# claymore666/openhush

Measured on AMD Instinct MI355X. Metric: audio-sec/sec (xRT) large-v3 greedy, 30s chunks, 1/2/4/8 MI355X, higher is better.
Workload: dtype bf16; 1 GPU; large-v3 dims, steps of batch=32 x 30 s windows per GPU, greedy, 100 tokens/window (EOT suppressed), procedural weights seed 1234, every window a distinct synthetic recording, PCM resident in HBM; schedule LANES 4x3: 12 steps (384 windows) in flight per GPU - per lane ONE front-end pass and ONE decode batch of 96 rows, 4 decodes side by side on 64 CUs each; concurrent_sub_batches=1

## Files before the change

### include/ohw.h

```cpp
#ifndef OHW_H
#define OHW_H

#include <stddef.h>
#include <stdint.h>

#ifdef __cplusplus
extern "C" {
#endif

#define OHW_ABI_VERSION 2

enum {
  OHW_OK = 0,
  OHW_E_MODEL_NOT_FOUND = -3001,
  OHW_E_LOAD_FAILED = -3002,
  OHW_E_TRANSCRIBE = -3003,
  OHW_E_NO_GPU = -3004,
  OHW_E_OOM = -3005,
  OHW_E_INVALID_ARG = -3006,
  OHW_E_VALIDATION = -3007
};

enum { OHW_DTYPE_AUTO = -1, OHW_DTYPE_BF16 = 0, OHW_DTYPE_F16 = 1 };

// ... 512 lines not shown
  void* x16_out;
  float* stat_out;
  void* k_cache;
  void* v_cache;
  const int32_t* n_past;
  int32_t d_model, n_head, n_ctx;
  int32_t* shape_out;
} ohw_dbg_dec_gemm_io;
int ohw_dbg_dec_gemm(const ohw_dbg_dec_gemm_io* io, void* stream);
int ohw_dbg_embed(int dtype, const float* emb, int n_vocab, const float* pos, int n_pos, const int32_t* tok_host,
                  const int32_t* n_past_host, float* x, void* x16, float* stat, int M, int n_new, int d, void* stream);
int ohw_dbg_layernorm(int dtype, const float* x, const float* gamma, const float* beta, void* y, int64_t rows, int d, int tiled,
                      void* stream);

enum { OHW_EG_KERNEL_AUTO = 0, OHW_EG_KERNEL_K128, OHW_EG_KERNEL_SMALL, OHW_EG_KERNEL_K256 };
typedef struct {
  int32_t dtype, epilogue, kernel;
  int32_t conv_cin;
  int64_t M, N, K;
  int64_t lda, a_batch_stride, rows_per_batch;
  int64_t ldc, c_batch_stride;
  int32_t d_model, n_head, t_len, batch, batch_offset;
  const int32_t* c_row_map;
  const void* a;
  int64_t a_elems;
  const float* w;
  const float* bias;
  const float* pos;
  void* out;
  int64_t out_elems;
} ohw_dbg_enc_gemm_io;
int ohw_dbg_enc_gemm(const ohw_dbg_enc_gemm_io* io, void* stream);

#ifdef __cplusplus
}
#endif
#endif
```

### openhush_amd/csrc/engine.hip

```cpp
#include <execinfo.h>
#include <signal.h>
#include <unistd.h>

#include <cstring>
#include <memory>
#include <mutex>
#include <shared_mutex>
#include <type_traits>
#include <vector>
#include <algorithm>

#include "attention.hpp"
#include "dequant.hpp"
#include "gemm.hpp"
#include "kernels.hpp"
#include "model.hpp"

namespace ohw {
ohw_ctx* ctx_from_file(const char* path, int device, int dtype);
ohw_ctx* ctx_synthetic(const ohw_hparams* hp, uint32_t seed, int device, int dtype);
ohw_ctx* ctx_shell(const ohw_hparams* hp, int device, int dtype);
void select_device(int device);

thread_local std::string g_last_error;
// ... 3180 lines not shown
      const int64_t need = (nb - 1) * a.c_batch_stride + (rows - 1) * a.ldc + a.N;
      if (need > a.out_elems) bad("the output rows end at element " + str(need) + ", past out_elems = " + str(a.out_elems));
      if (a.epilogue == EPI_GELU_POS_F32 && (!a.pos || !aligned16(a.pos))) bad("GELU_POS_F32 needs pos, 16-byte aligned");
    }

    hipStream_t s = (hipStream_t)stream;
    DevBuf wt, map;
    wt.alloc((size_t)a.N * a.K * 2);
    if (a.c_row_map) dbg_upload(map, a.c_row_map, (size_t)a.M);
    Dispatch::run(a.dtype, [&](auto* tag) {
      using TT = std::remove_pointer_t<decltype(tag)>;
      if (a.conv_cin > 0) launch_repack_conv<TT>(a.w, wt.p, a.N, a.conv_cin, a.K / 3, s);
      else launch_convert_rows<TT>(a.w, wt.p, a.N, a.K, a.K, s);
      GemmParams g{};
      g.A = a.a; g.W = wt.p; g.bias = a.bias; g.out = a.out; g.pos = a.epilogue == EPI_GELU_POS_F32 ? a.pos : nullptr;
      g.M = a.M; g.N = a.N; g.K = a.K;
      g.lda = a.lda; g.a_batch_stride = a.a_batch_stride; g.rows_per_batch = a.rows_per_batch;
      g.ldc = a.ldc; g.c_batch_stride = a.c_batch_stride;
      if (a.epilogue == EPI_CROSSKV_T) {
        g.d_model = a.d_model; g.n_head = a.n_head; g.t_len = a.t_len; g.batch = a.batch; g.batch_offset = a.batch_offset;
        g.c_row_map = a.c_row_map ? map.as<int32_t>() : nullptr;
      }
      switch (a.kernel) {
        case OHW_EG_KERNEL_K128: launch_gemm128<TT>(g, a.epilogue, s); break;
        case OHW_EG_KERNEL_SMALL: launch_gemm_small<TT>(g, a.epilogue, s); break;
        case OHW_EG_KERNEL_K256: launch_gemm256<TT>(g, a.epilogue, s); break;
        default: launch_gemm<TT>(g, a.epilogue, s); break;
      }
    });
    HIP_CHECK(hipStreamSynchronize(s));
  });
}

}
```

### openhush_amd/csrc/gemm.hpp

```cpp
#pragma once
#include "common.hpp"

namespace ohw {

enum GemmEpilogue {
  EPI_BIAS_T = 0,
  EPI_BIAS_GELU_T = 1,
  EPI_BIAS_RESID_F32 = 2,
  EPI_GELU_POS_F32 = 3,
  EPI_F32 = 4,
  EPI_CROSSKV_T = 5
};

struct GemmParams {
  const void* A;
  const void* W;
  const float* bias;
  void* out;
  const float* pos;
  int64_t M, N, K;
  int64_t lda, a_batch_stride, rows_per_batch;
  int64_t ldc, c_batch_stride;
  int32_t d_model, n_head, t_len, batch;
  int32_t batch_offset;
  int32_t group_m;
  int32_t small_m;
  const int32_t* c_row_map;
};

template <typename T> void launch_gemm(const GemmParams& p, int epilogue, hipStream_t stream);
template <typename T> void launch_gemm128(const GemmParams& p, int epilogue, hipStream_t stream);
template <typename T> void launch_gemm_small(const GemmParams& p, int epilogue, hipStream_t stream);
template <typename T> void launch_gemm256(const GemmParams& p, int epilogue, hipStream_t stream);

}
```

### openhush_amd/csrc/gemm256.hip

```cpp
#include <algorithm>
#include <cstdlib>

#include "gemm.hpp"
#include "gemm_epilogue.hpp"

namespace ohw {

constexpr int G2_BM = 256, G2_BN = 256, G2_BK = 64;
constexpr int G2_THREADS = 512;
constexpr int G2_OPSTAGE = 32768;
constexpr int G2_NA = 3;
constexpr int G2_WBASE = G2_NA * G2_OPSTAGE;
constexpr int G2_LDS = G2_WBASE + 2 * G2_OPSTAGE;

__device__ __forceinline__ int g2_key(int row) { return (row >> 1) & 7; }

#ifdef OHW_TRACE
constexpr unsigned G2_TRACE_CAP = 1u << 16;
__device__ unsigned long long g2_trace_buf[G2_TRACE_CAP * 12];
__device__ unsigned g2_trace_n;
#define G2T(k) do { if (tid == 0 && g2_slot < G2_TRACE_CAP) g2_trace_buf[g2_slot * 12 + (k)] = wall_clock64(); } while (0)
#else
#define G2T(k) do { } while (0)
#endif

template <typename T, int EPI>
__global__ __launch_bounds__(G2_THREADS, 2) void gemm256_kernel(GemmParams p) {
  using Ops = TypeOps<T>;
  using vec8 = typename Ops::vec8;
  extern __shared__ __attribute__((aligned(16))) unsigned char smem[];
  const int tid = threadIdx.x;
  const int lane = tid & 63;
  const int wave = __builtin_amdgcn_readfirstlane(tid >> 6);
  const int wm = wave >> 2, wn = wave & 3;
#ifdef OHW_TRACE
  unsigned g2_slot = G2_TRACE_CAP;
  if (tid == 0) {
    g2_slot = atomicAdd(&g2_trace_n, 1u);
    if (g2_slot < G2_TRACE_CAP) {
      unsigned hw, xcc;
      asm volatile("s_getreg_b32 %0, hwreg(HW_REG_HW_ID)" : "=s"(hw));
      asm volatile("s_getreg_b32 %0, hwreg(HW_REG_XCC_ID)" : "=s"(xcc));
      g2_trace_buf[g2_slot * 12 + 0] = blockIdx.x;
      g2_trace_buf[g2_slot * 12 + 1] = ((unsigned long long)(xcc & 0xf) << 32) | hw;
    }
  }
  G2T(2);
#endif

  const unsigned n_tiles_n = (unsigned)(p.N / G2_BN);
  const unsigned n_tiles_m = (unsigned)((p.M + G2_BM - 1) / G2_BM);
  const unsigned nwg = n_tiles_n * n_tiles_m;
  const T* __restrict__ A = (const T*)p.A;
  const T* __restrict__ W = (const T*)p.W;

  const int sr = lane >> 3, sc = lane & 7;
  unsigned a_off[4], w_off[4];
  int64_t m0 = 0, n0 = 0;
  auto tile_setup = [&](unsigned d) {
    const unsigned lid = xcd_remap(d, nwg);
    const unsigned GM = (unsigned)p.group_m;
    const unsigned per_group = GM * n_tiles_n;
    const unsigned grp_id = lid / per_group, in_grp = lid % per_group;
    const unsigned g_first = grp_id * GM;
    const unsigned g_size = n_tiles_m - g_first < GM ? n_tiles_m - g_first : GM;
    m0 = (int64_t)(g_first + in_grp % g_size) * G2_BM;
    n0 = (int64_t)(in_grp / g_size) * G2_BN;
#pragma unroll
    for (int j = 0; j < 4; ++j) {
      const int R = (wave * 4 + j) * 8 + sr;
      const int dchunk = sc ^ g2_key(R);
      int64_t m = m0 + R;
      if (m > p.M - 1) m = p.M - 1;
      int64_t b = 0, rr = m;
      if (p.rows_per_batch < p.M) { const unsigned bb = (unsigned)m / (unsigned)p.rows_per_batch; b = bb; rr = m - (int64_t)bb * p.rows_per_batch; }
      a_off[j] = (unsigned)((b * p.a_batch_stride + rr * p.lda + dchunk * 8) * 2);
      const int rl = R & 63;
      const int nl = (((rl >> 2) & 3) << 4) + ((rl >> 4) << 2) + (rl & 3);
      w_off[j] = (unsigned)(((n0 + (R & ~63) + nl) * p.K + dchunk * 8) * 2);
    }
  };
  const int KT = (int)(p.K / G2_BK);

  auto issue_A = [&](int kt) {
    const unsigned koff = (unsigned)(kt * G2_BK * 2);
    const int buf = (kt % G2_NA) * G2_OPSTAGE;
#pragma unroll
    for (int j = 0; j < 4; ++j)
      __builtin_amdgcn_global_load_lds((const __attribute__((address_space(1))) void*)((const char*)A + (size_t)(a_off[j] + koff)),
                                       (__attribute__((address_space(3))) void*)(smem + buf + (wave * 4 + j) * 1024), 16, 0, 0);
  };
  auto issue_W = [&](int kt) {
    const unsigned koff = (unsigned)(kt * G2_BK * 2);
// ... 23 lines not shown
#pragma unroll
    for (int ni = 0; ni < 4; ++ni) fw[ni] = *(const vec8*)(smem + wcur + w_row + ch + ni * 2048);
#pragma unroll
    for (int mi = 0; mi < 8; ++mi) fa[mi] = *(const vec8*)(smem + acur + a_row + ch + mi * 2048);
  };
  auto compute = [&]() {
    __builtin_amdgcn_s_setprio(1);
#pragma unroll
    for (int mi = 0; mi < 8; ++mi)
#pragma unroll
      for (int ni = 0; ni < 4; ++ni) acc[mi][ni] = Ops::mfma16(fw[ni], fa[mi], acc[mi][ni]);
    __builtin_amdgcn_s_setprio(0);
  };
  auto open_even = [&](int Pn) {
    if (Pn < NP && (Pn & 1) == 0) {
      if ((Pn >> 1) + 1 < KT) asm volatile("s_waitcnt vmcnt(4)" ::: "memory");
      else asm volatile("s_waitcnt vmcnt(0)" ::: "memory");
    }
    asm volatile("s_waitcnt lgkmcnt(0)" ::: "memory");
    __builtin_amdgcn_s_barrier();
    __builtin_amdgcn_sched_barrier(0);
  };
  auto open_odd = [&]() {
    asm volatile("s_waitcnt lgkmcnt(0)" ::: "memory");
    __builtin_amdgcn_s_barrier();
    __builtin_amdgcn_sched_barrier(0);
  };
  auto raw_barrier = [&]() {
    asm volatile("s_waitcnt lgkmcnt(0)" ::: "memory");
    __builtin_amdgcn_s_barrier();
    __builtin_amdgcn_sched_barrier(0);
  };

  const unsigned d = blockIdx.x;
  tile_setup(d);
  issue_A(0); issue_W(0);
  if (KT > 1) issue_A(1);
  {
    const int64_t m0c = m0, n0c = n0;
    const int64_t nb = n0c + wn * 64 + fq * 16;
    f32x4 bias4[4] = {{0.f, 0.f, 0.f, 0.f}, {0.f, 0.f, 0.f, 0.f}, {0.f, 0.f, 0.f, 0.f}, {0.f, 0.f, 0.f, 0.f}};
    if (p.bias) {
#pragma unroll
      for (int j = 0; j < 4; ++j) bias4[j] = *(const f32x4*)(p.bias + nb + 4 * j);
    }
#pragma unroll
    for (int i = 0; i < 8; ++i)
#pragma unroll
      for (int j = 0; j < 4; ++j) acc[i][j] = (f32x4){0.f, 0.f, 0.f, 0.f};

    if (wm == 0) {
      for (int P = 0; P < NP; ++P) {
        open_even(P);
#ifdef OHW_TRACE
        if (P == 0) G2T(3);
#endif
        read_frags(P);
        if ((P & 1) == 0) issue_ahead(P >> 1);
        __builtin_amdgcn_sched_barrier(0);
        open_odd();
        compute();
        __builtin_amdgcn_sched_barrier(0);
      }
      open_even(NP);
    } else {
      open_even(0);
      for (int P = 0; P < NP; ++P) {
        open_odd();
        read_frags(P);
        if ((P & 1) == 0) issue_ahead(P >> 1);
        __builtin_amdgcn_sched_barrier(0);
        open_even(P + 1);
        compute();
        __builtin_amdgcn_sched_barrier(0);
      }
    }
    G2T(4);

    int lane_e = lane;
    asm volatile("" : "+v"(lane_e));
    const int fr_e = lane_e & 15, fq_e = lane_e >> 4;
    float bias[16];
#pragma unroll
    for (int j = 0; j < 16; ++j) bias[j] = bias4[j >> 2][j & 3];
    bool stored = false;
    if constexpr (EPI == EPI_BIAS_RESID_F32) {
      float* outf = (float*)p.out;
      auto row_ptr = [&](int r, int i) -> float* {
        int64_t m = m0c + (wave >> 2) * 128 + r * 64 + (wave & 3) * 16 + i;
        if (m > p.M - 1) m = p.M - 1;
        int64_t bb = 0, rr = m;
        if (p.rows_per_batch < p.M) { const unsigned q = (unsigned)m / (unsigned)p.rows_per_batch; bb = q; rr = m - (int64_t)q * p.rows_per_batch; }
        return outf + bb * p.c_batch_stride + rr * p.ldc + n0c + lane_e * 4;
      };
      auto to_lds = [&](int r) {
#pragma unroll
        for (int q = 0; q < 4; ++q) {
          const int row = wm * 64 + q * 16 + fr_e;
#pragma unroll
          for (int ni = 0; ni < 4; ++ni) {
            const int chunk = (wn * 16 + fq_e * 4 + ni) ^ (row & 15);
            f32x4 v4 = acc[4 * r + q][ni];
            v4.x += bias[4 * ni]; v4.y += bias[4 * ni + 1]; v4.z += bias[4 * ni + 2]; v4.w += bias[4 * ni + 3];
            *(f32x4*)(smem + row * 1024 + chunk * 16) = v4;
          }
        }
      };
      f32x4 old0[16], old1[16];
#pragma unroll
      for (int i = 0; i < 16; ++i) old0[i] = *(const f32x4*)row_ptr(0, i);
      G2T(6);
      to_lds(0);
      raw_barrier();
      G2T(7);
#pragma unroll
      for (int i = 0; i < 16; ++i) old1[i] = *(const f32x4*)row_ptr(1, i);
#pragma unroll
      for (int i = 0; i < 16; ++i) {
        const int lr = wave * 16 + i;
        if (m0c + (wave >> 2) * 128 + (wave & 3) * 16 + i >= p.M) continue;
        const f32x4 v4 = *(const f32x4*)(smem + lr * 1024 + ((lane_e ^ (lr & 15)) << 4));
        f32x4 o4 = old0[i];
        o4.x += v4.x; o4.y += v4.y; o4.z += v4.z; o4.w += v4.w;
        *(f32x4*)row_ptr(0, i) = o4;
      }
      G2T(8);
      raw_barrier();
      to_lds(1);
      raw_barrier();
      G2T(9);
      f32x4 v1[16];
#pragma unroll
      for (int i = 0; i < 16; ++i) {
        const int lr = wave * 16 + i;
        v1[i] = *(const f32x4*)(smem + lr * 1024 + ((lane_e ^ (lr & 15)) << 4));
      }
#pragma unroll
      for (int i = 0; i < 16; ++i) {
        if (m0c + (wave >> 2) * 128 + 64 + (wave & 3) * 16 + i >= p.M) continue;
        f32x4 o4 = old1[i];
        o4.x += v1[i].x; o4.y += v1[i].y; o4.z += v1[i].z; o4.w += v1[i].w;
        *(f32x4*)row_ptr(1, i) = o4;
      }
      G2T(10);
      G2T(11);
      stored = true;
    }
    if constexpr (EPI == EPI_BIAS_T || EPI == EPI_BIAS_GELU_T) {
      {
        G2T(9);
#pragma unroll
        for (int mi = 0; mi < 8; ++mi) {
          const int row = wm * 128 + mi * 16 + fr_e;
          float v[16];
#pragma unroll
          for (int ni = 0; ni < 4; ++ni)
#pragma unroll
            for (int j = 0; j < 4; ++j) v[ni * 4 + j] = acc[mi][ni][j] + bias[ni * 4 + j];
          if constexpr (EPI == EPI_BIAS_GELU_T) {
#pragma unroll
            for (int j = 0; j < 16; ++j) v[j] = gelu_erf(v[j]);
          }
          u32x4 lo, hi;
          lo.x = pack2<T>(v[0], v[1]); lo.y = pack2<T>(v[2], v[3]); lo.z = pack2<T>(v[4], v[5]); lo.w = pack2<T>(v[6], v[7]);
          hi.x = pack2<T>(v[8], v[9]); hi.y = pack2<T>(v[10], v[11]); hi.z = pack2<T>(v[12], v[13]); hi.w = pack2<T>(v[14], v[15]);
          const int c0 = wn * 8 + fq_e * 2;
          *(u32x4*)(smem + row * 512 + ((c0 ^ fr_e) << 4)) = lo;
          *(u32x4*)(smem + row * 512 + (((c0 + 1) ^ fr_e) << 4)) = hi;
        }
        G2T(7);
        raw_barrier();
        G2T(8);
        T* outp = (T*)p.out;
#pragma unroll
        for (int half = 0; half < 2; ++half) {
#pragma unroll
          for (int i = 0; i < 8; ++i) {
            const int r = half * 128 + wave * 16 + 2 * i + (lane_e >> 5);
            const int64_t m = m0c + r;
            if (m >= p.M) continue;
            int64_t bb = 0, rr = m;
            if (p.rows_per_batch < p.M) { const unsigned q = (unsigned)m / (unsigned)p.rows_per_batch; bb = q; rr = m - (int64_t)q * p.rows_per_batch; }
            const u32x4 d4 = *(const u32x4*)(smem + r * 512 + (((lane_e & 31) ^ (r & 15)) << 4));
            *(u32x4*)(outp + bb * p.c_batch_stride + rr * p.ldc + n0c + (lane_e & 31) * 8) = d4;
          }
        }
        stored = true;
      }
    }
    if (!stored) {
#pragma unroll
      for (int mi = 0; mi < 8; ++mi) {
        const int64_t m = m0c + wm * 128 + mi * 16 + fr_e;
        if (m >= p.M) continue;
        float v[16];
#pragma unroll
        for (int ni = 0; ni < 4; ++ni)
#pragma unroll
          for (int j = 0; j < 4; ++j) v[ni * 4 + j] = acc[mi][ni][j] + bias[ni * 4 + j];
        gemm_store_row<T, EPI>(p, m, n0c + wn * 64 + fq_e * 16, v);
      }
    }
#ifdef OHW_TRACE
    G2T(6 + (EPI == EPI_BIAS_RESID_F32 ? 5 : 0));
    asm volatile("s_waitcnt vmcnt(0)" ::: "memory");
    G2T(5);
#endif
  }
}

template <typename T, int EPI>
static void launch256_one(const GemmParams& p, hipStream_t stream) {
  const unsigned nwg = (unsigned)((p.N / G2_BN) * ((p.M + G2_BM - 1) / G2_BM));
  ensure_dynamic_lds((const void*)gemm256_kernel<T, EPI>, G2_LDS);
  GemmParams q = p;
  static const int gm_env = [] { const char* e = getenv("OHW_GEMM_GM"); return e ? atoi(e) : 0; }();
  q.group_m = gm_env > 0 ? gm_env : 6;
  hipLaunchKernelGGL((gemm256_kernel<T, EPI>), dim3(nwg), dim3(G2_THREADS), G2_LDS, stream, q);
  HIP_CHECK(hipGetLastError());
}

template <typename T>
void launch_gemm256(const GemmParams& p, int epilogue, hipStream_t stream) {
  if (p.M <= 0) return;
  if (p.N % G2_BN != 0 || p.K % G2_BK != 0 || p.lda % 8 != 0 || p.a_batch_stride % 8 != 0 || p.rows_per_batch <= 0 || p.M >= ((int64_t)1 << 31) || p.N >= ((int64_t)1 << 31))
    throw Error(OHW_E_INVALID_ARG, "gemm256: N must be a multiple of 256, K of 64, row strides of 8 elements");
  {
    const int64_t nb_ = (p.M + p.rows_per_batch - 1) / p.rows_per_batch;
    const int64_t a_bytes = ((nb_ - 1) * p.a_batch_stride + (std::min(p.M, p.rows_per_batch) + 2) * p.lda + p.K) * 2, w_bytes = p.N * p.K * 2;
    if (a_bytes >= ((int64_t)1 << 32) || w_bytes >= ((int64_t)1 << 32)) throw Error(OHW_E_INVALID_ARG, "gemm256: an operand spans 4 GiB or more");
  }
  switch (epilogue) {
    case EPI_BIAS_T: launch256_one<T, EPI_BIAS_T>(p, stream); break;
    case EPI_BIAS_GELU_T: launch256_one<T, EPI_BIAS_GELU_T>(p, stream); break;
    case EPI_BIAS_RESID_F32: launch256_one<T, EPI_BIAS_RESID_F32>(p, stream); break;
    case EPI_GELU_POS_F32: launch256_one<T, EPI_GELU_POS_F32>(p, stream); break;
    case EPI_F32: launch256_one<T, EPI_F32>(p, stream); break;
    case EPI_CROSSKV_T: launch256_one<T, EPI_CROSSKV_T>(p, stream); break;
    default: throw Error(OHW_E_INVALID_ARG, "gemm256: unknown epilogue");
  }
}

template void launch_gemm256<bf16_t>(const GemmParams&, int, hipStream_t);
template void launch_gemm256<f16_t>(const GemmParams&, int, hipStream_t);

}

#ifdef OHW_TRACE
extern "C" int ohw_dbg_gemm_trace_read(unsigned long long* out, int cap_records) {
  unsigned n = 0;
  if (hipDeviceSynchronize() != hipSuccess) return -1;
// ... 10 lines not shown
```

### openhush_amd/engine.py

```python
from __future__ import annotations

import ctypes as C
import dataclasses
import os
import time
from typing import List, Optional, Sequence, Tuple, Union

import numpy as np

_HERE = os.path.dirname(os.path.abspath(__file__))
LIB_PATH = os.environ.get("OHW_LIB") or os.path.join(_HERE, "libohw.so")

CHUNK_SAMPLES = 480000
CHUNK_FRAMES = 3000

OHW_DTYPE_AUTO, OHW_DTYPE_BF16, OHW_DTYPE_F16 = -1, 0, 1
OHW_MEL_REFLECT, OHW_MEL_ZERO_TAIL = 0, 1
OHW_WINDOW_FIXED, OHW_WINDOW_SEEK, OHW_WINDOW_FIXED_RECORDING_MEL = 0, 1, 2
OHW_SCHEDULE_SEQUENTIAL, OHW_SCHEDULE_PIPELINE, OHW_SCHEDULE_LANES = 0, 1, 2
EPI_BIAS_T, EPI_BIAS_GELU_T, EPI_BIAS_RESID_F32, EPI_F32 = 0, 1, 2, 4
XA_PLAIN, XA_SPLIT, XA_ROWS2, XA_ROWS3, XA_ROWS4, XA_GROUP2, XA_GROUP3, XA_GROUP4, XA_GROUP5, XA_GROUP_SPLIT = range(10)
SA_PLAIN, SA_SLOTS = 0, 1

OHW_E_MODEL_NOT_FOUND, OHW_E_LOAD_FAILED, OHW_E_TRANSCRIBE = -3001, -3002, -3003
# ... 306 lines not shown
    "ohw_engine_last_trace", "ohw_engine_set_schedule", "ohw_ctx_dtype",
    "ohw_beam_search", "ohw_encode_slice", "ohw_dsp_resample_sinc", "ohw_default_vad_config", "ohw_vad_state_new", "ohw_vad_state_free", "ohw_vad_state_update",
    "ohw_vad_state_is_speech", "ohw_vad_state_speech_start", "ohw_vad_state_reset", "ohw_vad_energy_engine", "ohw_vad_energy_engine_free",
    "ohw_vad_run",
    "ohw_pool_create", "ohw_pool_transcribe", "ohw_pool_last_text", "ohw_pool_last_tokens", "ohw_pool_last_quality",
    "ohw_dbg_counter", "ohw_dsp_denoise", "ohw_denoise_passthrough_engine", "ohw_preprocess_audio_ex", "ohw_pool_set_window_mode",
    "ohw_state_set_persistent", "ohw_pool_broadcast_note", "ohw_pool_create_synthetic", "ohw_pool_set_force_len", "ohw_pool_set_schedule", "ohw_engine_set_force_len",
    "ohw_pool_set_decode_policy", "ohw_pool_n_devices", "ohw_pool_broadcast_kind", "ohw_pool_engine", "ohw_pool_free",
    "ohw_rng_uniforms", "ohw_rng_discard_draws", "ohw_sample_pass", "ohw_dbg_sample_t", "ohw_engine_set_fallback_device",
    "ohw_pool_set_fallback_device", "ohw_dequantize_host", "ohw_dbg_dequantize",
    "ohw_state_set_audio_ctx", "ohw_state_audio_ctx", "ohw_audio_ctx_for", "ohw_engine_set_audio_ctx", "ohw_pool_set_audio_ctx", "ohw_dbg_gemm_small",
    "ohw_state_set_window_ctx", "ohw_state_window_ctx", "ohw_engine_transcribe_batch", "ohw_engine_batch_result", "ohw_batch_plan",
    "ohw_state_set_packed_encoder", "ohw_state_packed_encoder", "ohw_engine_set_packed_encoder", "ohw_pool_set_packed_encoder", "ohw_dbg_poison",
    "ohw_dbg_attention_var", "ohw_dbg_cross_attn", "ohw_dbg_self_attn",
    "ohw_engine_set_detect_language", "ohw_engine_last_language", "ohw_engine_transcribe_batch_lang", "ohw_pool_set_detect_language",
    "ohw_state_set_window_lang", "ohw_state_detect_window_lang", "ohw_state_window_lang", "ohw_lang_pick_host", "ohw_dbg_lang_pick",
    "ohw_state_set_align_heads", "ohw_state_align", "ohw_align_reduce_host", "ohw_dtw_host", "ohw_dbg_align_probs", "ohw_dbg_align_reduce",
    "ohw_dbg_dtw", "ohw_engine_set_word_timestamps", "ohw_engine_last_token_times", "ohw_engine_last_words", "ohw_engine_last_segments",
    "ohw_engine_batch_times", "ohw_word_starts_host", "ohw_segments_host",
    "ohw_pool_set_word_timestamps", "ohw_pool_last_token_times", "ohw_pool_last_words", "ohw_pool_last_segments",
    "ohw_dbg_beam_step", "ohw_beam_search_ex", "ohw_dbg_beam_step_ex", "ohw_dbg_beam_finish", "ohw_beam_finish_host",
    "ohw_engine_set_beam_size", "ohw_pool_set_beam_size",
    "ohw_dbg_cross_attn_chunk",
    "ohw_state_set_window_prompt", "ohw_state_window_prompt_len", "ohw_state_prefill", "ohw_tokenize_host", "ohw_tokenize", "ohw_prompt_clip_host",
    "ohw_engine_set_initial_prompt", "ohw_engine_set_initial_prompt_tokens", "ohw_pool_set_initial_prompt",
    "ohw_recording_set_slot", "ohw_mel_seek_slots", "ohw_seek_sched_new", "ohw_seek_sched_round", "ohw_seek_sched_advance", "ohw_seek_sched_free",
    "ohw_engine_transcribe_long_batch", "ohw_engine_long_batch_quality",
    "ohw_dbg_dec_gemm", "ohw_dbg_embed", "ohw_dbg_layernorm",
    "ohw_state_set_prefill_chunk", "ohw_state_prefill_chunk", "ohw_engine_set_prefill_chunk", "ohw_dbg_cross_attn_chunk_n",
    "ohw_engine_set_carry_context", "ohw_pool_set_carry_context", "ohw_engine_last_context", "ohw_engine_long_batch_context", "ohw_carry_step_host",
    "ohw_seq_eval_host", "ohw_needs_fallback_host",
    "ohw_sample_pass_n", "ohw_dbg_sample_group", "ohw_best_of_pick_host", "ohw_engine_set_best_of", "ohw_pool_set_best_of",
    "ohw_engine_last_candidates", "ohw_engine_last_candidate_logprobs", "ohw_batch_windows_host",
    "ohw_dbg_enc_gemm",
    "ohw_phrase_table_build_host", "ohw_phrase_boost_host", "ohw_state_set_phrase_table", "ohw_state_phrase_count", "ohw_dbg_phrase_boost",
    "ohw_engine_set_hot_phrases", "ohw_engine_set_hot_phrases_tokens", "ohw_pool_set_hot_phrases",
]


class WhisperError(RuntimeError):
    def __init__(self, code: int, msg: str):
        super().__init__(msg)
        self.code = code


class ModelNotFound(WhisperError):
    pass


class LoadFailed(WhisperError):
    pass


class TranscriptionFailed(WhisperError):
    pass


class ValidationFailed(WhisperError):
    def __init__(self, code: int, msg: str, info: Optional[AudioInfo] = None):
        super().__init__(code, msg)
        self.info = info
        self.kind = AUDIO_ERRORS.get(info.error, "?") if info is not None else "?"


_lib = None


# ... 186 lines not shown
        L.ohw_pool_free.restype = None
        L.ohw_state_fetch.argtypes = [vp, C.c_char_p, C.c_int, fp, C.c_int64]
        L.ohw_state_profile_begin.argtypes = [vp, C.c_int]
        L.ohw_state_profile_end.argtypes = [vp, C.POINTER(C.c_int64), C.POINTER(C.c_double), C.POINTER(C.c_double)]
        L.ohw_ctx_weight_digest.argtypes = [vp, C.c_int, C.c_char_p, C.POINTER(C.c_uint64)]
        L.ohw_dbg_gemm.argtypes = [C.c_int, vp, vp, vp, vp, C.c_int64, C.c_int64, C.c_int64, C.c_int, vp]
        L.ohw_dbg_attention.argtypes = [C.c_int, vp, vp, C.c_int, C.c_int, C.c_int, vp]
        L.ohw_dbg_gemm_small.argtypes = [C.c_int, vp, vp, vp, vp, C.c_int64, C.c_int64, C.c_int64, C.c_int, vp]
        L.ohw_dbg_attention_var.argtypes = [C.c_int, vp, vp, C.c_int, C.c_int, C.c_int, ip, ip, vp]
        L.ohw_dbg_cross_attn.argtypes = [C.c_int, vp, vp, vp, vp, C.c_int, C.c_int, C.c_int, C.c_int, C.c_int, C.c_int, ip, ip, vp, vp, C.c_int,
                                         C.POINTER(C.c_int), vp]
        L.ohw_dbg_cross_attn_chunk.argtypes = [C.c_int, vp, vp, vp, vp, C.c_int, C.c_int, C.c_int, ip, ip, vp]
        L.ohw_state_set_window_prompt.argtypes = [vp, ip, C.c_int, ip, C.c_int]
        L.ohw_state_window_prompt_len.argtypes = [vp, C.c_int]
        L.ohw_state_prefill.argtypes = [vp, C.c_int, ip]
        L.ohw_tokenize_host.argtypes = [C.c_char_p, ip, C.c_int, C.c_char_p, ip, C.c_int]
        L.ohw_tokenize.argtypes = [vp, C.c_char_p, ip, C.c_int]
        L.ohw_prompt_clip_host.argtypes = [ip, C.c_int, C.c_int, ip]
        L.ohw_engine_set_initial_prompt.argtypes = [vp, C.c_char_p]
        L.ohw_engine_set_initial_prompt_tokens.argtypes = [vp, ip, C.c_int]
        L.ohw_pool_set_initial_prompt.argtypes = [vp, C.c_char_p]
        L.ohw_engine_set_carry_context.argtypes = [vp, C.c_int]
        L.ohw_state_set_prefill_chunk.argtypes = [vp, C.c_int]
        L.ohw_state_prefill_chunk.argtypes = [vp]
        L.ohw_engine_set_prefill_chunk.argtypes = [vp, C.c_int]
        L.ohw_dbg_cross_attn_chunk_n.argtypes = [C.c_int, vp, vp, vp, vp, C.c_int, C.c_int, C.c_int, ip, ip, vp, C.c_int]
        L.ohw_pool_set_carry_context.argtypes = [vp, C.c_int]
        L.ohw_engine_last_context.argtypes = [vp, C.c_int, C.POINTER(C.POINTER(C.c_int32)), C.POINTER(C.c_int)]
        L.ohw_engine_long_batch_context.argtypes = [vp, C.c_int, C.c_int, C.POINTER(C.POINTER(C.c_int32)), C.POINTER(C.c_int)]
        L.ohw_carry_step_host.argtypes = [ip, C.POINTER(C.c_int), C.c_int, ip, C.c_int, C.c_float, C.c_int, ip, C.POINTER(C.c_int)]
        L.ohw_dbg_self_attn.argtypes = [C.c_int, vp, vp, vp, ip, vp, C.c_int, C.c_int, C.c_int, C.c_int, ip, C.POINTER(C.c_int), vp]
        L.ohw_dbg_dec_gemm.argtypes = [C.POINTER(DbgDecGemmIO), vp]
        L.ohw_dbg_enc_gemm.argtypes = [C.POINTER(DbgEncGemmIO), vp]
        L.ohw_dbg_embed.argtypes = [C.c_int, vp, C.c_int, vp, C.c_int, ip, ip, vp, vp, vp, C.c_int, C.c_int, C.c_int, vp]
        L.ohw_dbg_layernorm.argtypes = [C.c_int, vp, vp, vp, vp, C.c_int64, C.c_int, C.c_int, vp]
        L.ohw_state_set_audio_ctx.argtypes = [vp, C.c_int]
        L.ohw_state_audio_ctx.argtypes = [vp]
        L.ohw_audio_ctx_for.argtypes = [C.c_int64]
        L.ohw_audio_ctx_for.restype = C.c_int32
        L.ohw_engine_set_audio_ctx.argtypes = [vp, C.c_int]
        L.ohw_pool_set_audio_ctx.argtypes = [vp, C.c_int]
        L.ohw_state_set_window_ctx.argtypes = [vp, C.POINTER(C.c_int32), C.c_int]
        L.ohw_state_window_ctx.argtypes = [vp, C.c_int]
        L.ohw_state_set_packed_encoder.argtypes = [vp, C.c_int]
        L.ohw_state_packed_encoder.argtypes = [vp]
        L.ohw_engine_set_packed_encoder.argtypes = [vp, C.c_int]
        L.ohw_pool_set_packed_encoder.argtypes = [vp, C.c_int]
        L.ohw_dbg_poison.argtypes = [vp, C.c_char_p]
        L.ohw_engine_transcribe_batch.argtypes = [vp, C.POINTER(AudioSpan), C.c_int, C.c_uint32]
        L.ohw_engine_batch_result.argtypes = [vp, C.c_int, C.POINTER(C.c_char_p), C.POINTER(C.c_size_t), C.POINTER(C.POINTER(C.c_int32)),
                                              C.POINTER(C.c_int), C.POINTER(C.POINTER(WindowQuality)), C.c_char_p]
        L.ohw_batch_plan.argtypes = [C.POINTER(C.c_int64), C.c_int, C.c_int, C.c_int, C.POINTER(C.c_int32), C.POINTER(C.c_int32),
                                     C.POINTER(C.c_int32)]
        L.ohw_engine_set_detect_language.argtypes = [vp, C.c_int]
        L.ohw_engine_last_language.argtypes = [vp, ip, fp]
        L.ohw_engine_transcribe_batch_lang.argtypes = [vp, C.POINTER(AudioSpan), ip, C.c_int, C.c_uint32]
        L.ohw_pool_set_detect_language.argtypes = [vp, C.c_int]
        L.ohw_state_set_window_lang.argtypes = [vp, C.POINTER(C.c_int32), C.c_int]
        L.ohw_state_detect_window_lang.argtypes = [vp, C.c_int]
        L.ohw_state_window_lang.argtypes = [vp, C.c_int, ip, fp]
        L.ohw_lang_pick_host.argtypes = [fp, C.POINTER(SpecialTokens), ip, fp]
        L.ohw_dbg_lang_pick.argtypes = [vp, fp, C.c_int, ip, fp]
        L.ohw_dbg_counter.argtypes = [vp, C.c_char_p]
        L.ohw_phrase_table_build_host.argtypes = [ip, ip, fp, C.c_int, C.c_int, vp]
        L.ohw_phrase_boost_host.argtypes = [vp, ip, C.c_int, fp, C.c_int]
        L.ohw_state_set_phrase_table.argtypes = [vp, ip, ip, fp, C.c_int]
# ... 188 lines not shown
def _spans(p, n, text_bytes: bytes):
    return [{"text": text_bytes[p[i].text_off:p[i].text_off + p[i].text_len].decode("utf-8", "replace"), "text_off": int(p[i].text_off),
             "text_len": int(p[i].text_len), "t0": float(p[i].t0), "t1": float(p[i].t1)} for i in range(n)]


def audio_ctx_for(n_samples: int) -> int:
    pos = (max(int(n_samples), 0) + 319) // 320 + 32
    return min(1500, (pos + 63) // 64 * 64)


def _audio_ctx_arg(n) -> int:
    if n is None:
        return 0
    if isinstance(n, str):
        if n.strip().lower() == "auto":
            return -1
        n = int(n)
    if int(n) < -1:
        raise ValueError("audio_ctx must be 0 (off), a positive context or \"auto\"")
    return int(n)


def batch_plan(n_samples: Sequence[int], max_batch: int, audio_ctx=0):
    ns = np.asarray(list(n_samples), dtype=np.int64)
    n = int(ns.size)
    order = np.zeros(max(n, 1), dtype=np.int32)
    ctx = np.zeros(max(n, 1), dtype=np.int32)
    env = np.zeros(max((n + max(int(max_batch), 1) - 1) // max(int(max_batch), 1), 1), dtype=np.int32)
    _check(lib().ohw_batch_plan(ns.ctypes.data_as(C.POINTER(C.c_int64)), n, int(max_batch), _audio_ctx_arg(audio_ctx), _ip(order), _ip(ctx),
                                _ip(env)))
    return order[:n].tolist(), ctx[:n].tolist(), env.tolist()


def last_error() -> str:
    return lib().ohw_last_error().decode("utf-8", "replace")


def _raise(code: int, info: Optional[AudioInfo] = None):
    msg = last_error()
    if code == OHW_E_MODEL_NOT_FOUND:
        raise ModelNotFound(code, msg)
    if code == OHW_E_VALIDATION:
        raise ValidationFailed(code, msg, info)
    if code in (OHW_E_LOAD_FAILED, OHW_E_NO_GPU, OHW_E_OOM):
        raise LoadFailed(code, msg)
    raise TranscriptionFailed(code, msg)


def _check(code: int):
    if code != 0:
        _raise(code)


def _fp(a: np.ndarray):
    assert a.dtype == np.float32 and a.flags["C_CONTIGUOUS"]
    return a.ctypes.data_as(C.POINTER(C.c_float))


def _ip(a: np.ndarray):
    assert a.dtype == np.int32 and a.flags["C_CONTIGUOUS"]
    return a.ctypes.data_as(C.POINTER(C.c_int32))


def validate_audio(samples: np.ndarray, sample_rate: int) -> AudioInfo:
    s = np.ascontiguousarray(samples, dtype=np.float32)
    info = AudioInfo()
# ... 1473 lines not shown
```

Measured before the change: 4034 audio-sec/sec.

## Make gemm256 persistent with per-XCD atomic tile stealing and epilogue prefetch overlap

The 256x256 encoder GEMM becomes persistent when not under graph capture. It launches as many workgroups as fit on the stream's CU mask, and each workgroup pulls further tiles from per-XCD atomic counters, stealing from other XCDs once its own is empty. The next tile's A/W loads are issued during the current tile's epilogue, using a second LDS staging region so the two can overlap. The aim is to cut wave-quantisation tails and launch imbalance when four lanes share 64 CUs each, at the cost of an extra memset, atomics and more complex LDS indexing.

```diff
diff --git a/include/ohw.h b/include/ohw.h
--- a/include/ohw.h
+++ b/include/ohw.h
@@ -568,6 +568,8 @@
 } ohw_dbg_enc_gemm_io;
 int ohw_dbg_enc_gemm(const ohw_dbg_enc_gemm_io* io, void* stream);
 
+int ohw_dbg_gemm256_forms(int persist, int max_wg);
+
 #ifdef __cplusplus
 }
 #endif
diff --git a/openhush_amd/csrc/engine.hip b/openhush_amd/csrc/engine.hip
--- a/openhush_amd/csrc/engine.hip
+++ b/openhush_amd/csrc/engine.hip
@@ -3236,4 +3236,11 @@
   });
 }
 
-}
+int ohw_dbg_gemm256_forms(int persist, int max_wg) {
+  return guard([&] {
+    if (persist > 2 || max_wg > (1 << 20)) throw Error(OHW_E_INVALID_ARG, "dbg_gemm256_forms: persist 0, 1 or 2 (negative: the environment's), max_wg at most 2^20");
+    gemm256_set_forms(persist, max_wg);
+  });
+}
+
+}
diff --git a/openhush_amd/csrc/gemm.hpp b/openhush_amd/csrc/gemm.hpp
--- a/openhush_amd/csrc/gemm.hpp
+++ b/openhush_amd/csrc/gemm.hpp
@@ -24,6 +24,7 @@
   int32_t d_model, n_head, t_len, batch;
   int32_t batch_offset;
   int32_t group_m;
+  uint32_t* tile_ctr;
   int32_t small_m;
   const int32_t* c_row_map;
 };
@@ -32,5 +33,6 @@
 template <typename T> void launch_gemm128(const GemmParams& p, int epilogue, hipStream_t stream);
 template <typename T> void launch_gemm_small(const GemmParams& p, int epilogue, hipStream_t stream);
 template <typename T> void launch_gemm256(const GemmParams& p, int epilogue, hipStream_t stream);
+void gemm256_set_forms(int persist, int max_wg);
 
 }
diff --git a/openhush_amd/csrc/gemm256.hip b/openhush_amd/csrc/gemm256.hip
--- a/openhush_amd/csrc/gemm256.hip
+++ b/openhush_amd/csrc/gemm256.hip
@@ -1,5 +1,7 @@
 #include <algorithm>
 #include <cstdlib>
+#include <mutex>
+#include <unordered_map>
 
 #include "gemm.hpp"
 #include "gemm_epilogue.hpp"
@@ -33,20 +35,6 @@
   const int lane = tid & 63;
   const int wave = __builtin_amdgcn_readfirstlane(tid >> 6);
   const int wm = wave >> 2, wn = wave & 3;
-#ifdef OHW_TRACE
-  unsigned g2_slot = G2_TRACE_CAP;
-  if (tid == 0) {
-    g2_slot = atomicAdd(&g2_trace_n, 1u);
-    if (g2_slot < G2_TRACE_CAP) {
-      unsigned hw, xcc;
-      asm volatile("s_getreg_b32 %0, hwreg(HW_REG_HW_ID)" : "=s"(hw));
-      asm volatile("s_getreg_b32 %0, hwreg(HW_REG_XCC_ID)" : "=s"(xcc));
-      g2_trace_buf[g2_slot * 12 + 0] = blockIdx.x;
-      g2_trace_buf[g2_slot * 12 + 1] = ((unsigned long long)(xcc & 0xf) << 32) | hw;
-    }
-  }
-  G2T(2);
-#endif
 
   const unsigned n_tiles_n = (unsigned)(p.N / G2_BN);
   const unsigned n_tiles_m = (unsigned)((p.M + G2_BM - 1) / G2_BM);
@@ -57,8 +45,7 @@
   const int sr = lane >> 3, sc = lane & 7;
   unsigned a_off[4], w_off[4];
   int64_t m0 = 0, n0 = 0;
-  auto tile_setup = [&](unsigned d) {
-    const unsigned lid = xcd_remap(d, nwg);
+  auto tile_setup = [&](unsigned lid) {
     const unsigned GM = (unsigned)p.group_m;
     const unsigned per_group = GM * n_tiles_n;
     const unsigned grp_id = lid / per_group, in_grp = lid % per_group;
@@ -148,11 +135,65 @@
     __builtin_amdgcn_sched_barrier(0);
   };
 
-  const unsigned d = blockIdx.x;
-  tile_setup(d);
+  unsigned* const ctr = p.tile_ctr;
+  const bool loop_tiles = ctr != nullptr;
+  const unsigned G = gridDim.x;
+  const unsigned xq = nwg / 8, xr = nwg % 8;
+  auto xcnt = [&](unsigned x) { return xq + (x < xr ? 1u : 0u); };
+  auto xbase = [&](unsigned x) { return x < xr ? x * (xq + 1) : xr * (xq + 1) + (x - xr) * xq; };
+  auto xfirst = [&](unsigned x) { return G / 8 + (x < G % 8 ? 1u : 0u); };
+  constexpr unsigned NO_TILE = 0xffffffffu;
+  unsigned cur_x = 0;
+  if (loop_tiles) {
+    unsigned xcc;
+    asm volatile("s_getreg_b32 %0, hwreg(HW_REG_XCC_ID)" : "=s"(xcc));
+    cur_x = xcc & 7;
+  }
+  constexpr int g2_word = (EPI == EPI_BIAS_RESID_F32 || EPI == EPI_BIAS_T || EPI == EPI_BIAS_GELU_T) ? G2_WBASE : 2 * G2_OPSTAGE;
+  unsigned drawn = 0;
+  unsigned nxt = NO_TILE;
+  auto publish_next = [&]() {
+    if (!loop_tiles || tid != 0) return;
+    unsigned t = NO_TILE, i = drawn;
+    for (unsigned tries = 0;;) {
+      if (i < xcnt(cur_x) - xfirst(cur_x)) { t = xbase(cur_x) + xfirst(cur_x) + i; break; }
+      if (++tries == 8) break;
+      cur_x = (cur_x + 1) & 7;
+      i = atomicAdd(&ctr[cur_x], 1u);
+    }
+    *(volatile unsigned*)(smem + g2_word) = t;
+  };
+  auto read_next = [&]() {
+    if (loop_tiles) nxt = __builtin_amdgcn_readfirstlane(*(volatile const unsigned*)(smem + g2_word));
+  };
+  auto next_tile = [&](bool behind_barrier) {
+    if (!loop_tiles || nxt == NO_TILE) return;
+    if (behind_barrier) raw_barrier();
+    tile_setup(nxt);
+    issue_A(0); issue_W(0);
+    if (KT > 1) issue_A(1);
+  };
+
+  tile_setup(xcd_remap(blockIdx.x, nwg));
   issue_A(0); issue_W(0);
   if (KT > 1) issue_A(1);
-  {
+#pragma unroll 1
+  for (;;) {
+#ifdef OHW_TRACE
+    unsigned g2_slot = G2_TRACE_CAP;
+    if (tid == 0) {
+      g2_slot = atomicAdd(&g2_trace_n, 1u);
+      if (g2_slot < G2_TRACE_CAP) {
+        unsigned hw, xcc;
+        asm volatile("s_getreg_b32 %0, hwreg(HW_REG_HW_ID)" : "=s"(hw));
+        asm volatile("s_getreg_b32 %0, hwreg(HW_REG_XCC_ID)" : "=s"(xcc));
+        g2_trace_buf[g2_slot * 12 + 0] = blockIdx.x;
+        g2_trace_buf[g2_slot * 12 + 1] = ((unsigned long long)(xcc & 0xf) << 32) | hw;
+      }
+    }
+    G2T(2);
+#endif
+    if (loop_tiles && tid == 0) drawn = atomicAdd(&ctr[cur_x], 1u);
     const int64_t m0c = m0, n0c = n0;
     const int64_t nb = n0c + wn * 64 + fq * 16;
     f32x4 bias4[4] = {{0.f, 0.f, 0.f, 0.f}, {0.f, 0.f, 0.f, 0.f}, {0.f, 0.f, 0.f, 0.f}, {0.f, 0.f, 0.f, 0.f}};
@@ -209,6 +250,7 @@
         if (p.rows_per_batch < p.M) { const unsigned q = (unsigned)m / (unsigned)p.rows_per_batch; bb = q; rr = m - (int64_t)q * p.rows_per_batch; }
         return outf + bb * p.c_batch_stride + rr * p.ldc + n0c + lane_e * 4;
       };
+      auto img = [&](int row) { return row * 1024 + (row >= 96 ? G2_OPSTAGE : 0); };
       auto to_lds = [&](int r) {
 #pragma unroll
         for (int q = 0; q < 4; ++q) {
@@ -218,7 +260,7 @@
             const int chunk = (wn * 16 + fq_e * 4 + ni) ^ (row & 15);
             f32x4 v4 = acc[4 * r + q][ni];
             v4.x += bias[4 * ni]; v4.y += bias[4 * ni + 1]; v4.z += bias[4 * ni + 2]; v4.w += bias[4 * ni + 3];
-            *(f32x4*)(smem + row * 1024 + chunk * 16) = v4;
+            *(f32x4*)(smem + img(wm * 64 + q * 16) + fr_e * 1024 + chunk * 16) = v4;
           }
         }
       };
@@ -226,8 +268,10 @@
 #pragma unroll
       for (int i = 0; i < 16; ++i) old0[i] = *(const f32x4*)row_ptr(0, i);
       G2T(6);
+      publish_next();
       to_lds(0);
       raw_barrier();
+      read_next();
       G2T(7);
 #pragma unroll
       for (int i = 0; i < 16; ++i) old1[i] = *(const f32x4*)row_ptr(1, i);
@@ -235,7 +279,7 @@
       for (int i = 0; i < 16; ++i) {
         const int lr = wave * 16 + i;
         if (m0c + (wave >> 2) * 128 + (wave & 3) * 16 + i >= p.M) continue;
-        const f32x4 v4 = *(const f32x4*)(smem + lr * 1024 + ((lane_e ^ (lr & 15)) << 4));
+        const f32x4 v4 = *(const f32x4*)(smem + img(lr) + ((lane_e ^ (lr & 15)) << 4));
         f32x4 o4 = old0[i];
         o4.x += v4.x; o4.y += v4.y; o4.z += v4.z; o4.w += v4.w;
         *(f32x4*)row_ptr(0, i) = o4;
@@ -249,14 +293,15 @@
 #pragma unroll
       for (int i = 0; i < 16; ++i) {
         const int lr = wave * 16 + i;
-        v1[i] = *(const f32x4*)(smem + lr * 1024 + ((lane_e ^ (lr & 15)) << 4));
-      }
+        v1[i] = *(const f32x4*)(smem + img(lr) + ((lane_e ^ (lr & 15)) << 4));
+      }
+#pragma unroll
+      for (int i = 0; i < 16; ++i) { v1[i].x += old1[i].x; v1[i].y += old1[i].y; v1[i].z += old1[i].z; v1[i].w += old1[i].w; }
+      next_tile(true);
 #pragma unroll
       for (int i = 0; i < 16; ++i) {
         if (m0c + (wave >> 2) * 128 + 64 + (wave & 3) * 16 + i >= p.M) continue;
-        f32x4 o4 = old1[i];
-        o4.x += v1[i].x; o4.y += v1[i].y; o4.z += v1[i].z; o4.w += v1[i].w;
-        *(f32x4*)row_ptr(1, i) = o4;
+        *(f32x4*)row_ptr(1, i) = v1[i];
       }
       G2T(10);
       G2T(11);
@@ -264,10 +309,10 @@
     }
     if constexpr (EPI == EPI_BIAS_T || EPI == EPI_BIAS_GELU_T) {
       {
+        auto img16 = [&](int row) { return row * 512 + (row >= 192 ? G2_OPSTAGE : 0); };
         G2T(9);
 #pragma unroll
         for (int mi = 0; mi < 8; ++mi) {
-          const int row = wm * 128 + mi * 16 + fr_e;
           float v[16];
 #pragma unroll
           for (int ni = 0; ni < 4; ++ni)
@@ -281,11 +326,13 @@
           lo.x = pack2<T>(v[0], v[1]); lo.y = pack2<T>(v[2], v[3]); lo.z = pack2<T>(v[4], v[5]); lo.w = pack2<T>(v[6], v[7]);
           hi.x = pack2<T>(v[8], v[9]); hi.y = pack2<T>(v[10], v[11]); hi.z = pack2<T>(v[12], v[13]); hi.w = pack2<T>(v[14], v[15]);
           const int c0 = wn * 8 + fq_e * 2;
-          *(u32x4*)(smem + row * 512 + ((c0 ^ fr_e) << 4)) = lo;
-          *(u32x4*)(smem + row * 512 + (((c0 + 1) ^ fr_e) << 4)) = hi;
+          *(u32x4*)(smem + img16(wm * 128 + mi * 16) + fr_e * 512 + ((c0 ^ fr_e) << 4)) = lo;
+          *(u32x4*)(smem + img16(wm * 128 + mi * 16) + fr_e * 512 + (((c0 + 1) ^ fr_e) << 4)) = hi;
         }
         G2T(7);
+        publish_next();
         raw_barrier();
+        read_next();
         G2T(8);
         T* outp = (T*)p.out;
 #pragma unroll
@@ -297,14 +344,21 @@
             if (m >= p.M) continue;
             int64_t bb = 0, rr = m;
             if (p.rows_per_batch < p.M) { const unsigned q = (unsigned)m / (unsigned)p.rows_per_batch; bb = q; rr = m - (int64_t)q * p.rows_per_batch; }
-            const u32x4 d4 = *(const u32x4*)(smem + r * 512 + (((lane_e & 31) ^ (r & 15)) << 4));
+            const u32x4 d4 = *(const u32x4*)(smem + img16(half * 128 + wave * 16) + (2 * i + (lane_e >> 5)) * 512 + (((lane_e & 31) ^ (r & 15)) << 4));
             *(u32x4*)(outp + bb * p.c_batch_stride + rr * p.ldc + n0c + (lane_e & 31) * 8) = d4;
           }
+          if (half == 0) next_tile(true);
         }
         stored = true;
       }
     }
     if (!stored) {
+      if (loop_tiles) {
+        publish_next();
+        raw_barrier();
+        read_next();
+        next_tile(false);
+      }
 #pragma unroll
       for (int mi = 0; mi < 8; ++mi) {
         const int64_t m = m0c + wm * 128 + mi * 16 + fr_e;
@@ -319,10 +373,45 @@
     }
 #ifdef OHW_TRACE
     G2T(6 + (EPI == EPI_BIAS_RESID_F32 ? 5 : 0));
-    asm volatile("s_waitcnt vmcnt(0)" ::: "memory");
+    if (!loop_tiles || nxt == NO_TILE) asm volatile("s_waitcnt vmcnt(0)" ::: "memory");
     G2T(5);
 #endif
-  }
+    if (!loop_tiles || nxt == NO_TILE) break;
+  }
+}
+
+static int g2_persist_override = -1, g2_max_wg = 0;
+static int g2_persist() {
+  static const int env = [] { const char* e = getenv("OHW_GEMM_PERSIST"); return e ? atoi(e) : 1; }();
+  const int v = __atomic_load_n(&g2_persist_override, __ATOMIC_RELAXED);
+  return v >= 0 ? v : env;
+}
+void gemm256_set_forms(int persist, int max_wg) {
+  __atomic_store_n(&g2_persist_override, persist < 0 ? -1 : persist, __ATOMIC_RELAXED);
+  __atomic_store_n(&g2_max_wg, max_wg > 0 ? max_wg : 0, __ATOMIC_RELAXED);
+}
+
+struct G2Stream { uint32_t* ctr = nullptr; int cus = 0; };
+static G2Stream g2_stream(hipStream_t stream) {
+  static std::mutex mu;
+  static std::unordered_map<hipStream_t, G2Stream> known;
+  std::lock_guard<std::mutex> lock(mu);
+  auto it = known.find(stream);
+  if (it != known.end()) return it->second;
+  G2Stream g;
+  HIP_CHECK(hipMalloc((void**)&g.ctr, 64));
+  uint32_t mask[16] = {0};
+  if (stream && hipExtStreamGetCUMask(stream, 16, mask) == hipSuccess) {
+    int n = 0, total = 0, dev = 0;
+    for (uint32_t m : mask) n += __builtin_popcount(m);
+    (void)hipGetDevice(&dev);
+    (void)hipDeviceGetAttribute(&total, hipDeviceAttributeMultiprocessorCount, dev);
+    if (n > 0 && n < total) g.cus = n;
+  } else {
+    (void)hipGetLastError();
+  }
+  known.emplace(stream, g);
+  return g;
 }
 
 template <typename T, int EPI>
@@ -332,7 +421,24 @@
   GemmParams q = p;
   static const int gm_env = [] { const char* e = getenv("OHW_GEMM_GM"); return e ? atoi(e) : 0; }();
   q.group_m = gm_env > 0 ? gm_env : 6;
-  hipLaunchKernelGGL((gemm256_kernel<T, EPI>), dim3(nwg), dim3(G2_THREADS), G2_LDS, stream, q);
+  unsigned grid = nwg;
+  q.tile_ctr = nullptr;
+  hipStreamCaptureStatus cap = hipStreamCaptureStatusNone;
+  const int mode = g2_persist();
+  if ((mode >= 2 || (mode == 1 && p.N / G2_BN > 5)) && hipStreamIsCapturing(stream, &cap) == hipSuccess && cap == hipStreamCaptureStatusNone) {
+    static const int per_cu = [] { int n = 0; if (hipOccupancyMaxActiveBlocksPerMultiprocessor(&n, (const void*)gemm256_kernel<T, EPI>, G2_THREADS, G2_LDS) != hipSuccess) { (void)hipGetLastError(); n = 1; } return std::max(n, 1); }();
+    static const int n_cu = [] { int dev = 0, n = 0; (void)hipGetDevice(&dev); (void)hipDeviceGetAttribute(&n, hipDeviceAttributeMultiprocessorCount, dev); return n > 0 ? n : 256; }();
+    const G2Stream gs = g2_stream(stream);
+    unsigned want = (unsigned)per_cu * (unsigned)(gs.cus > 0 ? gs.cus : n_cu);
+    const int cap_wg = __atomic_load_n(&g2_max_wg, __ATOMIC_RELAXED);
+    if (cap_wg > 0) want = std::min(want, (unsigned)cap_wg);
+    if (want < nwg) {
+      grid = want;
+      q.tile_ctr = gs.ctr;
+      HIP_CHECK(hipMemsetAsync(gs.ctr, 0, 64, stream));
+    }
+  }
+  hipLaunchKernelGGL((gemm256_kernel<T, EPI>), dim3(grid), dim3(G2_THREADS), G2_LDS, stream, q);
   HIP_CHECK(hipGetLastError());
 }
 
diff --git a/openhush_amd/engine.py b/openhush_amd/engine.py
--- a/openhush_amd/engine.py
+++ b/openhush_amd/engine.py
@@ -362,7 +362,7 @@
     "ohw_seq_eval_host", "ohw_needs_fallback_host",
     "ohw_sample_pass_n", "ohw_dbg_sample_group", "ohw_best_of_pick_host", "ohw_engine_set_best_of", "ohw_pool_set_best_of",
     "ohw_engine_last_candidates", "ohw_engine_last_candidate_logprobs", "ohw_batch_windows_host",
-    "ohw_dbg_enc_gemm",
+    "ohw_dbg_enc_gemm", "ohw_dbg_gemm256_forms",
     "ohw_phrase_table_build_host", "ohw_phrase_boost_host", "ohw_state_set_phrase_table", "ohw_state_phrase_count", "ohw_dbg_phrase_boost",
     "ohw_engine_set_hot_phrases", "ohw_engine_set_hot_phrases_tokens", "ohw_pool_set_hot_phrases",
 ]
@@ -615,6 +615,7 @@
         L.ohw_dbg_self_attn.argtypes = [C.c_int, vp, vp, vp, ip, vp, C.c_int, C.c_int, C.c_int, C.c_int, ip, C.POINTER(C.c_int), vp]
         L.ohw_dbg_dec_gemm.argtypes = [C.POINTER(DbgDecGemmIO), vp]
         L.ohw_dbg_enc_gemm.argtypes = [C.POINTER(DbgEncGemmIO), vp]
+        L.ohw_dbg_gemm256_forms.argtypes = [C.c_int, C.c_int]
         L.ohw_dbg_embed.argtypes = [C.c_int, vp, C.c_int, vp, C.c_int, ip, ip, vp, vp, vp, C.c_int, C.c_int, C.c_int, vp]
         L.ohw_dbg_layernorm.argtypes = [C.c_int, vp, vp, vp, vp, C.c_int64, C.c_int, C.c_int, vp]
         L.ohw_state_set_audio_ctx.argtypes = [vp, C.c_int]
@@ -869,6 +870,10 @@
     return order[:n].tolist(), ctx[:n].tolist(), env.tolist()
 
 
+def dbg_gemm256_forms(persist: int = -1, max_wg: int = 0) -> None:
+    _check(lib().ohw_dbg_gemm256_forms(int(persist), int(max_wg)))
+
+
 def last_error() -> str:
     return lib().ohw_last_error().decode("utf-8", "replace")
 
```

New measurement: 4051 audio-sec/sec, median of 3. No clear change (+0.4%).
